# wjmaddox/online_gp

Measured on AMD Instinct MI355X. Metric: streaming updates/sec (WISKI, 50^3 inducing grid), higher is better.
Workload: dtype f32

## Files before the change

online_gp_amd/csrc/scatter_owner.h:

```cpp
#pragma once

template <typename real>
struct OwnerRec {
  static constexpr int N = 16;
};

__device__ __forceinline__ float wave_readlane(float v, int src) { return __builtin_bit_cast(float, __builtin_amdgcn_readlane(__builtin_bit_cast(int, v), src)); }
__device__ __forceinline__ int wave_readlane(int v, int src) { return __builtin_amdgcn_readlane(v, src); }
__device__ __forceinline__ double wave_readlane(double v, int src) {
  const long long b = __builtin_bit_cast(long long, v);
  const int lo = __builtin_amdgcn_readlane((int)(b & 0xffffffffll), src), hi = __builtin_amdgcn_readlane((int)(b >> 32), src);
  return __builtin_bit_cast(double, ((long long)hi << 32) | (long long)(unsigned)lo);
}
__device__ __forceinline__ void lds_atomic_add(float* p, float v) { __hip_atomic_fetch_add(p, v, __ATOMIC_RELAXED, __HIP_MEMORY_SCOPE_WORKGROUP); }
__device__ __forceinline__ void lds_atomic_add(double* p, double v) { __hip_atomic_fetch_add(p, v, __ATOMIC_RELAXED, __HIP_MEMORY_SCOPE_WORKGROUP); }

template <typename real>
static inline int64_t owner_work_bytes(const wiski_grid* g, int64_t n) {
  const int64_t ncell = (int64_t)(g->g[0] - 3) * (g->g[1] - 3) * (g->g[2] - 3);
  const int64_t heads = (ncell * 8 + 255) / 256 * 256, next = (n * 4 + 255) / 256 * 256;
  return heads + next + n * OwnerRec<real>::N * (int64_t)sizeof(real);
}

template <typename real>
__global__ __launch_bounds__(256) void k_bin_points(GridDev<real> G, const real* __restrict__ x, const real* __restrict__ y, const real* __restrict__ wa,
                                                    const real* __restrict__ wb, const real* __restrict__ noise, int64_t n,
                                                    double* __restrict__ stats, int32_t* __restrict__ err, const real* __restrict__ u, int carry,
                                                    real* __restrict__ mean_out, unsigned long long* __restrict__ head, int32_t* __restrict__ next,
                                                    real* __restrict__ rec, unsigned epoch, uint32_t* __restrict__ z1, int64_t n1,
                                                    uint32_t* __restrict__ z2, int64_t n2, const long long* __restrict__ guard, long long guard_expect) {
  if (guard && *guard != guard_expect) return;
  for (int64_t e = (int64_t)blockIdx.x * blockDim.x + threadIdx.x; e < n1; e += (int64_t)gridDim.x * blockDim.x) z1[e] = 0u;
  for (int64_t e = (int64_t)blockIdx.x * blockDim.x + threadIdx.x; e < n2; e += (int64_t)gridDim.x * blockDim.x) z2[e] = 0u;
  __shared__ double s_red[16];
  const int lane = threadIdx.x & 63, loc = threadIdx.x >> 6;
  const int nc1 = G.g[1] - 3, nc2 = G.g[2] - 3;
  bool bad = false;
  for (int64_t base = (int64_t)blockIdx.x * 4; base < n; base += (int64_t)gridDim.x * 4) {
    const int64_t p = base + loc;
    if (p >= n) continue;
    real xp[3], w[3][4];
    int j0[3];
#pragma unroll
    for (int q = 0; q < 3; ++q) xp[q] = x[p * 3 + q];
    const bool inside = point_stencil<real, 3>(G, xp, j0, w);
    if (!inside) {
      bad = true;
      if (lane == 0) {
        atomicAdd(err, 2);
        next[p] = -2;
        if (mean_out) mean_out[p] = (real)0;
      }
      continue;
    }
    const int a = lane >> 4, b = (lane >> 2) & 3, c = lane & 3;
    const real wa_ = a == 0 ? w[0][0] : a == 1 ? w[0][1] : a == 2 ? w[0][2] : w[0][3];
    const real wb_ = b == 0 ? w[1][0] : b == 1 ? w[1][1] : b == 2 ? w[1][2] : w[1][3];
    const real wc_ = c == 0 ? w[2][0] : c == 1 ? w[2][1] : c == 2 ? w[2][2] : w[2][3];
    const real v = wa_ * wb_ * wc_;
    const int64_t flat = (int64_t)(j0[0] + a) * G.stride[0] + (int64_t)(j0[1] + b) * G.stride[1] + (j0[2] + c);
    real wu = (u && v != (real)0) ? v * u[flat] : (real)0;
    if (u) wu = wave_reduce_sum<real>(wu);
    {
      real wl = (real)0;
#pragma unroll
      for (int q = 0; q < 3; ++q)
#pragma unroll
        for (int k = 0; k < 4; ++k)
          if (lane == 4 * q + k) wl = w[q][k];
      if (lane < 12) rec[p * OwnerRec<real>::N + lane] = wl;
    }
    if (lane == 12) {
      const real wap = wa[p], by = y[p] * wb[p];
      real* r = rec + p * OwnerRec<real>::N;
      r[12] = wap;
      r[13] = by;
      r[14] = carry ? by - wap * wu : (real)0;
      r[15] = (real)0;
      if (mean_out) mean_out[p] = wu;
      const int64_t cell = ((int64_t)j0[0] * nc1 + j0[1]) * nc2 + j0[2];
      const unsigned long long tag = ((unsigned long long)epoch << 32) | (unsigned long long)(unsigned)p;
      const unsigned long long old = atomicExch(head + cell, tag);
      next[p] = (unsigned)(old >> 32) == epoch ? (int32_t)(old & 0xffffffffull) : -1;
    }
  }
  scatter_stats_pass<real, 3>(G, x, y, wb, noise, n, stats, s_red);
  if (bad) atomicOr(err, 1);
}

__device__ __forceinline__ int owner_slot(int g, int s) { return g == 0 ? s - 3 : 4 + 7 * (g - 1) + s; }

template <typename real, int NT>
__global__ __launch_bounds__(NT) void k_owner_lines(GridDev<real> G, real* __restrict__ A, real* __restrict__ b, real* __restrict__ cnt,
                                                     real* __restrict__ res, const unsigned long long* __restrict__ head,
                                                     const int32_t* __restrict__ next, const real* __restrict__ rec, unsigned epoch,
                                                     const long long* __restrict__ guard, long long guard_expect, int abl) {
  if (guard && *guard != guard_expect) return;
  extern __shared__ __attribute__((aligned(16))) char smem_owner[];
  constexpr int NS = 172;
  const int g0 = G.g[0], g1 = G.g[1], g2 = G.g[2];
  const int nc0 = g0 - 3, nc1 = g1 - 3, nc2 = g2 - 3;
  const int i0 = blockIdx.x / g1, i1 = blockIdx.x % g1;
  real* acc = reinterpret_cast<real*>(smem_owner);
  real* vb = acc + (size_t)g2 * NS;
  real* vc = vb + g2;
  real* vr = vc + g2;
  __shared__ int s_any;
  const int t = threadIdx.x, lane = t & 63, wv = t >> 6;
  {
    const int nz = g2 * (NS + 3), nz4 = nz & ~3;
    for (int e = 4 * t; e < nz4; e += 4 * NT) {
      acc[e] = (real)0; acc[e + 1] = (real)0; acc[e + 2] = (real)0; acc[e + 3] = (real)0;
    }
    if (t < nz - nz4) acc[nz4 + t] = (real)0;
  }
  if (t == 0) s_any = 0;
  __syncthreads();
  const int lo = g2 * wv / (NT / 64), hi = g2 * (wv + 1) / (NT / 64);
  const int clo = lo - 3 < 0 ? 0 : lo - 3, chi = hi < nc2 ? hi : nc2;
  const int ncw = chi - clo, ncand = 16 * ncw;
  const unsigned inv_ncw = (65536u + (unsigned)ncw - 1u) / (unsigned)ncw;
  int found = 0;
  const int a = lane >> 4, bq = (lane >> 2) & 3, c = lane & 3;
  const int dummy = g2 * (NS + 3) + t;
  real m0[4], m1[4], m2[4];
#pragma unroll
  for (int k = 0; k < 4; ++k) {
    m0[k] = a == k ? (real)1 : (real)0;
    m1[k] = bq == k ? (real)1 : (real)0;
    m2[k] = c == k ? (real)1 : (real)0;
  }
  const int lcode = 7 * a + bq;
  const int lidx = 7 * lcode + c;
  auto visit = [&](real (&r)[15], int p, int da, int db, int c2) {
    const int dcode = 7 * da + db;
    const bool upper = lcode > dcode, same = lcode == dcode;
    const int abase = lidx + (c2 * NS - 7 * dcode);
    for (;;) {
      const real w0a = m0[0] * r[0] + m0[1] * r[1] + m0[2] * r[2] + m0[3] * r[3];
      const real w1b = m1[0] * r[4] + m1[1] * r[5] + m1[2] * r[6] + m1[3] * r[7];
      const real w2c = m2[0] * r[8] + m2[1] * r[9] + m2[2] * r[10] + m2[3] * r[11];
      const real w0d = da == 0 ? r[0] : da == 1 ? r[1] : da == 2 ? r[2] : r[3];
      const real w1d = db == 0 ? r[4] : db == 1 ? r[5] : db == 2 ? r[6] : r[7];
      const real wab = w0d * w1d;
      const real wj = w0a * w1b * w2c;
      const real wap = r[12];
      int ix[7];
      real add[7], cur[7];
      const real wpj = wap * wab * wj;
#pragma unroll
      for (int cr = 0; cr < 4; ++cr) {
        const bool keep = (upper || (same && c >= cr)) && c2 + cr >= lo && c2 + cr < hi;
        ix[cr] = keep ? abase + cr * (NS - 1) : dummy;
        add[cr] = wpj * r[8 + cr];
      }
      {
        const bool mine = lane < 4 && c2 + lane >= lo && c2 + lane < hi;
        const real wi = wab * w2c;
        const int row = g2 * NS + c2 + lane;
        ix[4] = mine ? row : dummy;
        ix[5] = mine ? row + g2 : dummy;
        ix[6] = mine ? row + 2 * g2 : dummy;
        add[4] = wi * r[13];
        add[5] = wi * wap;
        add[6] = wi * r[14];
      }
#pragma unroll
      for (int k = 0; k < 7; ++k) cur[k] = acc[ix[k]];
#pragma unroll
      for (int k = 0; k < 7; ++k) acc[ix[k]] = cur[k] + add[k];
      if (p < 0) break;
      const real* __restrict__ rp = rec + (int64_t)p * OwnerRec<real>::N;
#pragma unroll
      for (int k = 0; k < 15; ++k) r[k] = rp[k];
      p = next[p];
    }
  };
  constexpr int RB = sizeof(real) == 4 ? 5 : 3;
  for (int cb0 = 0; cb0 < ncand; cb0 += 64 * RB) {
    int p0[RB], nx[RB];
    real rl[RB][15];
#pragma unroll
    for (int rb = 0; rb < RB; ++rb) {
      const int ci = cb0 + 64 * rb + lane;
      p0[rb] = -1;
      if (ci < ncand) {
        const int dd = (int)(((unsigned)ci * inv_ncw) >> 16), c2 = clo + ci - dd * ncw;
        const int c0 = i0 - (dd >> 2), c1 = i1 - (dd & 3);
        if (c0 >= 0 && c0 < nc0 && c1 >= 0 && c1 < nc1) {
          const unsigned long long h = head[((int64_t)c0 * nc1 + c1) * nc2 + c2];
          if ((unsigned)(h >> 32) == epoch) p0[rb] = (int)(unsigned)(h & 0xffffffffull);
        }
      }
    }
#pragma unroll
    for (int rb = 0; rb < RB; ++rb) {
      nx[rb] = -1;
      if (p0[rb] >= 0) {
        const real* __restrict__ r = rec + (int64_t)p0[rb] * OwnerRec<real>::N;
#pragma unroll
        for (int k = 0; k < 15; ++k) rl[rb][k] = r[k];
        nx[rb] = next[p0[rb]];
      } else {
#pragma unroll
        for (int k = 0; k < 15; ++k) rl[rb][k] = (real)0;
      }
    }
#pragma unroll
    for (int rb = 0; rb < RB; ++rb) {
      unsigned long long live = __ballot(p0[rb] >= 0);
      if (abl & 1) { found |= live != 0; live = 0; }
      while (live) {
        const int src = __ffsll((long long)live) - 1;
        live &= live - 1;
        const int ci_s = cb0 + 64 * rb + src;
        const int dd = __builtin_amdgcn_readfirstlane((int)(((unsigned)ci_s * inv_ncw) >> 16));
        const int c2 = __builtin_amdgcn_readfirstlane(clo + ci_s - dd * ncw);
        found = 1;
        real r[15];
#pragma unroll
        for (int k = 0; k < 15; ++k) r[k] = wave_readlane(rl[rb][k], src);
        visit(r, wave_readlane(nx[rb], src), dd >> 2, dd & 3, c2);
      }
    }
  }
  if (found && lane == 0) s_any = 1;
  __syncthreads();
  if (!s_any || (abl & 2)) return;
  const int64_t m = G.m;
  const int64_t row0 = ((int64_t)i0 * g1 + i1) * g2;
  {
    const int n0 = 4 * g2;
    for (int e = t; e < n0; e += NT) {
      const real v = acc[(e >> 2) * NS + (e & 3)];
      if (v != (real)0) A[row0 * 4 + e] += v;
    }
  }
  const int n1 = 7 * g2;
  constexpr int NE = (448 + NT - 1) / NT;
  bool ok[NE];
  int le[NE];
#pragma unroll
  for (int j = 0; j < NE; ++j) {
    const int e = t + NT * j;
    ok[j] = e < n1;
    le[j] = (e / 7) * NS + 4 + (e % 7);
  }
  constexpr int GB = NE <= 2 ? 6 : 3;
  for (int gq = 0; gq < 24; gq += GB) {
    real v[GB][NE], o[GB][NE];
#pragma unroll
    for (int k = 0; k < GB; ++k)
#pragma unroll
      for (int j = 0; j < NE; ++j) v[k][j] = ok[j] ? acc[le[j] + 7 * (gq + k)] : (real)0;
#pragma unroll
    for (int k = 0; k < GB; ++k) {
      const real* __restrict__ Ag = A + (int64_t)(7 * (gq + k + 1) - 3) * m + row0 * 7;
#pragma unroll
      for (int j = 0; j < NE; ++j) o[k][j] = *(v[k][j] != (real)0 ? Ag + t + NT * j : A);
    }
#pragma unroll
    for (int k = 0; k < GB; ++k) {
      real* __restrict__ Ag = A + (int64_t)(7 * (gq + k + 1) - 3) * m + row0 * 7;
#pragma unroll
      for (int j = 0; j < NE; ++j)
        if (v[k][j] != (real)0) {
#ifdef WISKI_OWNER_NT_STORES
          __builtin_nontemporal_store(o[k][j] + v[k][j], Ag + t + NT * j);
#else
          Ag[t + NT * j] = o[k][j] + v[k][j];
#endif
        }
    }
  }
  for (int e = t; e < g2; e += NT) {
    if (vb[e] != (real)0) b[row0 + e] += vb[e];
    if (cnt && vc[e] != (real)0) cnt[row0 + e] += vc[e];
    if (res && vr[e] != (real)0) res[row0 + e] += vr[e];
  }
}
```

online_gp_amd/csrc/scatter_stats.hip:

```cpp
#include "wiski_common.h"

#ifndef WISKI_SCATTER_ATOMIC_MOD
#define WISKI_SCATTER_ATOMIC_MOD 0
#endif
__device__ __forceinline__ void stencil_atomic(float* p, float v) {
#if WISKI_SCATTER_ATOMIC_MOD == 1
  asm volatile("global_atomic_add_f32 %0, %1, off sc1" ::"v"(p), "v"(v) : "memory");
#elif WISKI_SCATTER_ATOMIC_MOD == 2
  asm volatile("global_atomic_add_f32 %0, %1, off nt" ::"v"(p), "v"(v) : "memory");
#elif WISKI_SCATTER_ATOMIC_MOD == 3
  asm volatile("global_atomic_add_f32 %0, %1, off sc1 nt" ::"v"(p), "v"(v) : "memory");
#else
  unsafeAtomicAdd(p, v);
#endif
}
__device__ __forceinline__ void stencil_atomic(double* p, double v) { unsafeAtomicAdd(p, v); }
#include <atomic>
#include <cstdlib>

struct ScatterBatch {
  int64_t y_stride = 0, w_stride = 0, vec_stride = 0, A_stride = 0;
};

template <typename real, int D>
__device__ __forceinline__ void scatter_stats_pass(const GridDev<real>& G, const real* __restrict__ x, const real* __restrict__ y,
                                                   const real* __restrict__ wb, const real* __restrict__ noise, int64_t n,
                                                   double* __restrict__ stats, double* s_red) {
  int64_t want = n / 512;
  want = want < 1 ? 1 : (want > 64 ? 64 : want);
  const int ns = (int64_t)gridDim.x < want ? (int)gridDim.x : (int)want;
  if ((int)blockIdx.x >= ns) return;
  double c_acc = 0, ld_acc = 0;
  for (int64_t p = (int64_t)blockIdx.x * blockDim.x + threadIdx.x; p < n; p += (int64_t)ns * blockDim.x) {
    real xp[D], w[D][4];
    int j0[D];
#pragma unroll
    for (int q = 0; q < D; ++q) xp[q] = x[p * D + q];
    if (point_stencil<real, D>(G, xp, j0, w)) {
      const double yp = (double)y[p];
      c_acc += yp * yp * (double)wb[p];
      ld_acc += log((double)noise[p]);
    }
  }
  const double c_tot = block_reduce_sum(c_acc, s_red);
  const double ld_tot = block_reduce_sum(ld_acc, s_red);
  if (threadIdx.x == 0 && (c_tot != 0 || ld_tot != 0)) {
    unsafeAtomicAdd(stats + 0, c_tot);
    unsafeAtomicAdd(stats + 1, ld_tot);
  }
}

template <typename real, int D>
__global__ __launch_bounds__(256) void k_scatter_stats(GridDev<real> G, const real* __restrict__ x, const real* __restrict__ y,
                                                       const real* __restrict__ wa, const real* __restrict__ wb,
                                                       const real* __restrict__ noise, int64_t n, real* __restrict__ b,
                                                       real* __restrict__ A_st, double* __restrict__ stats, int32_t* __restrict__ err,
                                                       real* __restrict__ cnt) {
  constexpr int T = 1 << (2 * D);
  constexpr int GRP = T < 64 ? T : 64;
  constexpr int PPB = 256 / GRP;
  constexpr int TPL = T / GRP;
  __shared__ real s_val[PPB][T];
  __shared__ double s_red[16];
  const int sub = threadIdx.x % GRP;
  const int loc = threadIdx.x / GRP;
  int R = 1;
#pragma unroll
  for (int q = 0; q < D; ++q) R *= 7;
  const int center = (R - 1) / 2;
  bool bad = false;

  for (int64_t base = (int64_t)blockIdx.x * PPB; base < n; base += (int64_t)gridDim.x * PPB) {
    const int64_t p = base + loc;
    const bool valid = p < n;
    int j0[D];
    real w[D][4];
    real yp = 0, wap = 0, wbp = 0;
    if (valid) {
      real xp[D];
#pragma unroll
      for (int q = 0; q < D; ++q) xp[q] = x[p * D + q];
      const bool inside = point_stencil<real, D>(G, xp, j0, w);
      if (!inside) {
        bad = true;
        if (sub == 0) atomicAdd(err, 2);
      }
      yp = y[p];
      wap = wa[p];
      wbp = wb[p];
    } else {
#pragma unroll
      for (int q = 0; q < D; ++q) {
        j0[q] = 0;
#pragma unroll
        for (int c = 0; c < 4; ++c) w[q][c] = 0;
      }
    }
    int idx_a[TPL], code_a[TPL];
    real val_a[TPL];
#pragma unroll
    for (int t = 0; t < TPL; ++t) {
      const int a = sub + t * GRP;
      int flat = 0, code = 0;
      real v = (real)1;
#pragma unroll
      for (int q = 0; q < D; ++q) {
        const int c = (a >> (2 * (D - 1 - q))) & 3;
        flat += (j0[q] + c) * G.stride[q];
        code = code * 7 + c;
        v *= w[q][c];
      }
      idx_a[t] = flat;
      code_a[t] = code;
      val_a[t] = v;
      s_val[loc][a] = v;
    }
    __syncthreads();
    if (valid) {
#pragma unroll
      for (int t = 0; t < TPL; ++t) {
        if (val_a[t] != (real)0) {
          atomic_add_real(b + idx_a[t], val_a[t] * yp * wbp);
          if (cnt) atomic_add_real(cnt + idx_a[t], val_a[t] * wap);
          if (A_st) {
            const real va = val_a[t] * wap;
            real* __restrict__ Arow = A_st + idx_a[t];
            const int obase = center - code_a[t];
#pragma unroll 4
            for (int bb0 = 0; bb0 < T; ++bb0) {
              const int bb = (bb0 & ~3) | ((bb0 + (sub + t * GRP)) & 3);
              int codeb = 0;
#pragma unroll
              for (int q = 0; q < D; ++q) codeb = codeb * 7 + ((bb >> (2 * (D - 1 - q))) & 3);
              const real vb = s_val[loc][bb];
              if (vb != (real)0) atomic_add_real(Arow + (int64_t)(obase + codeb) * G.m, va * vb);
            }
          }
        }
      }
    }
    __syncthreads();
  }
  scatter_stats_pass<real, D>(G, x, y, wb, noise, n, stats, s_red);
  if (bad) atomicOr(err, 1);
}

template <typename real, int D>
__global__ __launch_bounds__(256) void k_scatter_stats_sym(GridDev<real> G, const real* __restrict__ x, const real* __restrict__ y,
                                                           const real* __restrict__ wa, const real* __restrict__ wb,
                                                           const real* __restrict__ noise, int64_t n, real* __restrict__ b,
                                                           real* __restrict__ A, double* __restrict__ stats, int32_t* __restrict__ err,
                                                           real* __restrict__ cnt, const real* __restrict__ u, real* __restrict__ res,
                                                           real* __restrict__ mean_out = nullptr, uint32_t* __restrict__ z1 = nullptr,
                                                           int64_t n1 = 0, uint32_t* __restrict__ z2 = nullptr, int64_t n2 = 0,
                                                           const long long* __restrict__ guard = nullptr, long long guard_expect = 0,
                                                           int g_lo = 0, int g_hi = 1 << 30, ScatterBatch bt = ScatterBatch{}) {
  {
    const int64_t o = blockIdx.y;
    y += o * bt.y_stride; wa += o * bt.w_stride; wb += o * bt.w_stride; noise += o * bt.w_stride;
    b += o * bt.vec_stride; stats += 2 * o;
    if (A) A += o * bt.A_stride;
    if (cnt) cnt += o * bt.vec_stride;
    if (u) u += o * bt.vec_stride;
    if (res) res += o * bt.vec_stride;
  }
  if (guard && *guard != guard_expect) return;
  for (int64_t e = (int64_t)blockIdx.x * blockDim.x + threadIdx.x; e < n1; e += (int64_t)gridDim.x * blockDim.x) z1[e] = 0u;
  for (int64_t e = (int64_t)blockIdx.x * blockDim.x + threadIdx.x; e < n2; e += (int64_t)gridDim.x * blockDim.x) z2[e] = 0u;
  constexpr int T = 1 << (2 * D);
  constexpr int TP = T / 4;
  constexpr int NPAIR = TP * (TP + 1) / 2;
  constexpr int TPL = T > 64 ? T / 64 : 1;
  __shared__ real s_val[4][T];
  __shared__ int s_idx[4][T];
  __shared__ int s_pair[NPAIR];
  __shared__ int s_scan[4];
  __shared__ double s_red[16];
  const int lane = threadIdx.x & 63, loc = threadIdx.x >> 6;
  int npair = 0;
  {
    int running = 0;
    for (int base = 0; base < TP * TP; base += 256) {
      const int idx = base + threadIdx.x;
      const int pa = idx / TP, pb = idx % TP;
      int ca = 0, cb = 0;
#pragma unroll
      for (int q = 0; q < D - 1; ++q) {
        ca = ca * 7 + ((pa >> (2 * (D - 2 - q))) & 3);
        cb = cb * 7 + ((pb >> (2 * (D - 2 - q))) & 3);
      }
      const bool ok = idx < TP * TP && cb >= ca && cb - ca >= g_lo && cb - ca < g_hi;
      const unsigned long long mask = __ballot(ok);
      if (lane == 0) s_scan[loc] = __popcll(mask);
      __syncthreads();
      int off = running;
      for (int w = 0; w < loc; ++w) off += s_scan[w];
      if (ok) s_pair[off + __popcll(mask & ((1ull << lane) - 1ull))] = pa | (pb << 8) | ((cb - ca) << 16);
      running += s_scan[0] + s_scan[1] + s_scan[2] + s_scan[3];
      __syncthreads();
    }
    npair = running;
  }
  bool bad = false;
  const int64_t m = G.m;
  for (int64_t base = (int64_t)blockIdx.x * 4; base < n; base += (int64_t)gridDim.x * 4) {
    const int64_t p = base + loc;
    const bool valid = p < n;
    int j0[D];
    real w[D][4];
    real yp = 0, wap = 0, wbp = 0;
    if (valid) {
      real xp[D];
#pragma unroll
      for (int q = 0; q < D; ++q) xp[q] = x[p * D + q];
      const bool inside = point_stencil<real, D>(G, xp, j0, w);
      if (!inside) {
        bad = true;
        if (lane == 0 && blockIdx.y == 0) atomicAdd(err, 2);
      }
      yp = y[p];
      wap = wa[p];
      wbp = wb[p];
    } else {
#pragma unroll
      for (int q = 0; q < D; ++q) {
        j0[q] = 0;
#pragma unroll
        for (int c = 0; c < 4; ++c) w[q][c] = 0;
      }
    }
    int flat_t[TPL];
    real val_t[TPL];
    real wu = (real)0;
#pragma unroll
    for (int t = 0; t < TPL; ++t) {
      const int a = lane + t * 64;
      flat_t[t] = 0;
      val_t[t] = (real)0;
      if (a < T) {
        int flat = 0;
        real v = (real)1;
#pragma unroll
        for (int q = 0; q < D; ++q) {
          const int c = (a >> (2 * (D - 1 - q))) & 3;
          flat += (j0[q] + c) * G.stride[q];
          v *= w[q][c];
        }
        s_val[loc][a] = v;
        s_idx[loc][a] = flat;
        flat_t[t] = flat;
        val_t[t] = v;
        if (u && v != (real)0) wu += v * u[flat];
      }
    }
    real innov = yp * wbp;
    if (u) {
#pragma unroll
      for (int off = 32; off > 0; off >>= 1) wu += __shfl_xor(wu, off, 64);
      innov -= wap * wu;
      if (mean_out && lane == 0 && valid) mean_out[p] = wu;
    }
#pragma unroll
    for (int t = 0; t < TPL; ++t) {
      if (valid && val_t[t] != (real)0) {
        atomic_add_real(b + flat_t[t], val_t[t] * yp * wbp);
        if (cnt) atomic_add_real(cnt + flat_t[t], val_t[t] * wap);
        if (res) atomic_add_real(res + flat_t[t], val_t[t] * innov);
      }
    }
    __syncthreads();
    if (valid && A) {
      const int a2 = lane & 3, b2 = (lane >> 2) & 3, ps = lane >> 4;
#pragma unroll 2
      for (int t0 = 0; t0 < npair; t0 += 4) {
        const int t = t0 + ps;
        if (t < npair) {
          const int pk = s_pair[t];
          const int g = pk >> 16;
          const int a = (pk & 0xff) * 4 + a2;
          const real v = wap * s_val[loc][a] * s_val[loc][((pk >> 8) & 0xff) * 4 + b2];
          const int64_t row = s_idx[loc][a];
          if (g == 0) {
            if (b2 >= a2 && v != (real)0) stencil_atomic(A + row * 4 + (b2 - a2), v);
          } else if (v != (real)0) {
            stencil_atomic(A + (int64_t)(7 * g - 3) * m + row * 7 + (b2 - a2 + 3), v);
          }
        }
      }
    }
    __syncthreads();
  }
  scatter_stats_pass<real, D>(G, x, y, wb, noise, n, stats, s_red);
  if (bad) atomicOr(err, 1);
}

#include "scatter_owner.h"

template <typename real>
__global__ __launch_bounds__(256) void k_stencil_expand_add(GridDev<real> G, real* __restrict__ half, real* __restrict__ full) {
  const int m = G.m, d = G.d;
  const int c = (G.R - 1) / 2;
  const int oh = blockIdx.y;
  int rem = c + oh, off = 0;
  for (int q = d - 1; q >= 0; --q) {
    off += (rem % 7 - 3) * G.stride[q];
    rem /= 7;
  }
  const int g = oh < 4 ? 0 : (oh - 4) / 7 + 1;
  real* __restrict__ h = oh < 4 ? half + oh : half + (int64_t)(7 * g - 3) * m + (oh - 4) % 7;
  const int hs = oh < 4 ? 4 : 7;
  real* __restrict__ fd = full + (int64_t)(c + oh) * m;
  real* __restrict__ fm = full + (int64_t)(c - oh) * m;
  for (int i = blockIdx.x * blockDim.x + threadIdx.x; i < m; i += gridDim.x * blockDim.x) {
    const real v = h[(int64_t)i * hs];
    if (v != (real)0) {
      fd[i] += v;
      if (oh > 0) {
        const int j = i + off;
        if (j >= 0 && j < m) fm[j] += v;
      }
      h[(int64_t)i * hs] = (real)0;
    }
  }
}

template <typename real>
static int expand_impl(const wiski_grid* grid, real* d_half, real* d_full, void* stream) {
  GridDev<real> G;
  int rc = make_grid_dev<real>(grid, &G);
  if (rc) return rc;
  if (!d_half || !d_full) return WISKI_E_BADARG;
  int bx = (G.m + 255) / 256;
  if (bx > 64) bx = 64;
  dim3 grd((unsigned)bx, (unsigned)((G.R + 1) / 2));
  hipLaunchKernelGGL((k_stencil_expand_add<real>), grd, dim3(256), 0, (hipStream_t)stream, G, d_half, d_full);
  WISKI_LAUNCH_CHECK();
  return WISKI_OK;
}

static int64_t owner_min_points() {
  static int64_t v = -1;
  if (v < 0) {
    const char* e = getenv("WISKI_OWNER_MIN_POINTS");
    v = e ? atoll(e) : 8192;
    if (v <= 0) v = (int64_t)1 << 62;
  }
  return v;
}

static int owner_ablate() { return 0; }

template <typename real>
static int scatter_impl(const wiski_grid* grid, const real* d_x, const real* d_y, const real* d_wa, const real* d_wb, const real* d_noise,
                        int64_t n, real* d_b, real* d_A_st, double* d_stats, int32_t* d_err, void* stream, bool half = false,
                        real* d_cnt = nullptr, const real* d_u = nullptr, real* d_res = nullptr, real* d_mean_out = nullptr,
                        void* z1 = nullptr, int64_t n1_bytes = 0, void* z2 = nullptr, int64_t n2_bytes = 0, const void* d_guard = nullptr,
                        int64_t guard_expect = 0, void* d_bin = nullptr, int64_t bin_bytes = 0, int g_lo = 0, int g_hi = 1 << 30, int nout = 1,
                        ScatterBatch bt = ScatterBatch{}) {
  GridDev<real> G;
  int rc = make_grid_dev<real>(grid, &G);
  if (rc) return rc;
  if (n == 0) return WISKI_OK;
  if (!d_x || !d_y || !d_wa || !d_wb || !d_noise || !d_b || !d_stats || !d_err) return WISKI_E_BADARG;
  if (d_mean_out == nullptr && (d_u != nullptr) != (d_res != nullptr)) return WISKI_E_BADARG;
  if ((d_res && !d_u) || (d_mean_out && !d_u) || (d_u && !half)) return WISKI_E_BADARG;
  if (d_guard && !half) return WISKI_E_BADARG;
  if ((n1_bytes | n2_bytes) & 3 || (n1_bytes && !z1) || (n2_bytes && !z2) || ((n1_bytes || n2_bytes) && !half)) return WISKI_E_BADARG;
  const bool ranged = g_lo > 0 || g_hi < (1 << 30);
  if (ranged && !half) return WISKI_E_BADARG;
  if (nout < 1 || (nout > 1 && (!half || d_mean_out || n1_bytes || n2_bytes || d_guard))) return WISKI_E_BADARG;
  bool owner = !ranged && nout == 1 && half && G.d == 3 && d_bin && d_cnt && d_A_st && G.g[2] <= 64 && G.g[0] > 3 && G.g[1] > 3 && G.g[2] > 3 && n < (int64_t)1 << 31 &&
               n >= owner_min_points() && bin_bytes >= owner_work_bytes<real>(grid, n);
  const size_t owner_lds = ((size_t)G.g[2] * (172 + 3) + 512) * sizeof(real);
  if (owner) {
    static int lds_max = -1;
    static size_t lds_set = 0;
    if (lds_max < 0) {
      int dev = 0, v = 0;
      if (hipGetDevice(&dev) != hipSuccess || hipDeviceGetAttribute(&v, hipDeviceAttributeMaxSharedMemoryPerBlock, dev) != hipSuccess) v = 64 * 1024;
      lds_max = v;
    }
    if (owner_lds > (size_t)lds_max) {
      owner = false;
    } else if (owner_lds > 48 * 1024 && owner_lds > lds_set) {
      if (hipFuncSetAttribute((const void*)k_owner_lines<real, 256>, hipFuncAttributeMaxDynamicSharedMemorySize, (int)owner_lds) != hipSuccess ||
          hipFuncSetAttribute((const void*)k_owner_lines<real, 128>, hipFuncAttributeMaxDynamicSharedMemorySize, (int)owner_lds) != hipSuccess ||
          hipFuncSetAttribute((const void*)k_owner_lines<real, 512>, hipFuncAttributeMaxDynamicSharedMemorySize, (int)owner_lds) != hipSuccess) {
        (void)hipGetLastError();
        owner = false;
      } else {
        lds_set = owner_lds;
      }
    }
  }
  if (owner) {
    static std::atomic<unsigned> epoch_src{0};
    unsigned epoch = ++epoch_src;
    if (!epoch) epoch = ++epoch_src;
    const int64_t ncell = (int64_t)(G.g[0] - 3) * (G.g[1] - 3) * (G.g[2] - 3);
    char* w = static_cast<char*>(d_bin);
    unsigned long long* head = reinterpret_cast<unsigned long long*>(w);
    int32_t* next = reinterpret_cast<int32_t*>(w + (ncell * 8 + 255) / 256 * 256);
    real* rec = reinterpret_cast<real*>(w + (ncell * 8 + 255) / 256 * 256 + (n * 4 + 255) / 256 * 256);
    int64_t nb = (n + 3) / 4;
    if (nb > 2048) nb = 2048;
    hipLaunchKernelGGL((k_bin_points<real>), dim3((unsigned)nb), dim3(256), 0, (hipStream_t)stream, G, d_x, d_y, d_wa, d_wb, d_noise, n, d_stats, d_err,
                       d_u, d_res != nullptr ? 1 : 0, d_mean_out, head, next, rec, epoch, (uint32_t*)z1, n1_bytes / 4, (uint32_t*)z2, n2_bytes / 4,
                       (const long long*)d_guard, (long long)guard_expect);
    constexpr int owner_nt = 256;
    const size_t lds = owner_lds;
    const int abl = owner_ablate();
    hipLaunchKernelGGL((k_owner_lines<real, owner_nt>), dim3((unsigned)(G.g[0] * G.g[1])), dim3(owner_nt), lds, (hipStream_t)stream, G, d_A_st, d_b, d_cnt, d_res,
                       (const unsigned long long*)head, (const int32_t*)next, (const real*)rec, epoch, (const long long*)d_guard, (long long)guard_expect, abl);
    return hipGetLastError() == hipSuccess ? WISKI_OK : WISKI_E_LAUNCH;
  }
  const int grp = half ? 64 : (G.T < 64 ? G.T : 64);
  const int64_t ppb = 256 / grp;
  int64_t blocks = (n + ppb - 1) / ppb;
  if (blocks > 256 * 8) blocks = 256 * 8;
  dim3 grd((unsigned)blocks, (unsigned)nout);
#define CALL(DD)                                                                                                                              \
  do {                                                                                                                                        \
    if (half) hipLaunchKernelGGL((k_scatter_stats_sym<real, DD>), grd, dim3(256), 0, (hipStream_t)stream, G, d_x, d_y, d_wa, d_wb, d_noise, n, d_b, d_A_st, d_stats, d_err, d_cnt, d_u, d_res, d_mean_out, (uint32_t*)z1, n1_bytes / 4, (uint32_t*)z2, n2_bytes / 4, (const long long*)d_guard, (long long)guard_expect, g_lo, g_hi, bt); \
    else hipLaunchKernelGGL((k_scatter_stats<real, DD>), grd, dim3(256), 0, (hipStream_t)stream, G, d_x, d_y, d_wa, d_wb, d_noise, n, d_b, d_A_st, d_stats, d_err, d_cnt);   \
  } while (0)
  WISKI_DISPATCH_D(G.d, CALL)
#undef CALL
  WISKI_LAUNCH_CHECK();
  return WISKI_OK;
}

extern "C" {
int wiski_scatter_stats_f32(const wiski_grid* g, const float* x, const float* y, const float* wa, const float* wb, const float* noise, int64_t n, float* b, float* A, double* stats, int32_t* err, void* s) {
  return scatter_impl<float>(g, x, y, wa, wb, noise, n, b, A, stats, err, s);
}
int wiski_scatter_stats_f64(const wiski_grid* g, const double* x, const double* y, const double* wa, const double* wb, const double* noise, int64_t n, double* b, double* A, double* stats, int32_t* err, void* s) {
  return scatter_impl<double>(g, x, y, wa, wb, noise, n, b, A, stats, err, s);
}
int wiski_scatter_stats_sym_f32(const wiski_grid* g, const float* x, const float* y, const float* wa, const float* wb, const float* noise, int64_t n, float* b, float* A_half, double* stats, int32_t* err, void* s) {
  return scatter_impl<float>(g, x, y, wa, wb, noise, n, b, A_half, stats, err, s, true);
}
int wiski_scatter_stats_sym_f64(const wiski_grid* g, const double* x, const double* y, const double* wa, const double* wb, const double* noise, int64_t n, double* b, double* A_half, double* stats, int32_t* err, void* s) {
  return scatter_impl<double>(g, x, y, wa, wb, noise, n, b, A_half, stats, err, s, true);
}
int wiski_scatter_stats_cnt_f32(const wiski_grid* g, const float* x, const float* y, const float* wa, const float* wb, const float* noise, int64_t n, float* b, float* A, int32_t half, float* cnt, const float* u, float* res, double* stats, int32_t* err, void* s) {
  return scatter_impl<float>(g, x, y, wa, wb, noise, n, b, A, stats, err, s, half != 0, cnt, u, res);
}
int wiski_scatter_stats_cnt_f64(const wiski_grid* g, const double* x, const double* y, const double* wa, const double* wb, const double* noise, int64_t n, double* b, double* A, int32_t half, double* cnt, const double* u, double* res, double* stats, int32_t* err, void* s) {
  return scatter_impl<double>(g, x, y, wa, wb, noise, n, b, A, stats, err, s, half != 0, cnt, u, res);
}
int wiski_scatter_stats_step_f32(const wiski_grid* g, const float* x, const float* y, const float* wa, const float* wb, const float* noise, int64_t n, float* b, float* A_half, float* cnt, const float* u, float* res, float* mean_out, double* stats, int32_t* err, void* z1, int64_t n1, void* z2, int64_t n2, const void* guard, int64_t guard_expect, void* bin, int64_t bin_bytes, void* s) {
  return scatter_impl<float>(g, x, y, wa, wb, noise, n, b, A_half, stats, err, s, true, cnt, u, res, mean_out, z1, n1, z2, n2, guard, guard_expect, bin, bin_bytes);
}
int wiski_scatter_stats_step_f64(const wiski_grid* g, const double* x, const double* y, const double* wa, const double* wb, const double* noise, int64_t n, double* b, double* A_half, double* cnt, const double* u, double* res, double* mean_out, double* stats, int32_t* err, void* z1, int64_t n1, void* z2, int64_t n2, const void* guard, int64_t guard_expect, void* bin, int64_t bin_bytes, void* s) {
  return scatter_impl<double>(g, x, y, wa, wb, noise, n, b, A_half, stats, err, s, true, cnt, u, res, mean_out, z1, n1, z2, n2, guard, guard_expect, bin, bin_bytes);
}
int wiski_scatter_stats_step_sharded_f32(const wiski_grid* g, const float* x, const float* y, const float* wa, const float* wb, const float* noise, int64_t n, float* b, float* A_half, float* cnt, const float* u, float* res, float* mean_out, double* stats, int32_t* err, void* z1, int64_t n1, void* z2, int64_t n2, const void* guard, int64_t guard_expect, int32_t g_lo, int32_t g_hi, void* s) {
  return scatter_impl<float>(g, x, y, wa, wb, noise, n, b, A_half, stats, err, s, true, cnt, u, res, mean_out, z1, n1, z2, n2, guard, guard_expect, nullptr, 0, g_lo, g_hi);
}
int wiski_scatter_stats_step_sharded_f64(const wiski_grid* g, const double* x, const double* y, const double* wa, const double* wb, const double* noise, int64_t n, double* b, double* A_half, double* cnt, const double* u, double* res, double* mean_out, double* stats, int32_t* err, void* z1, int64_t n1, void* z2, int64_t n2, const void* guard, int64_t guard_expect, int32_t g_lo, int32_t g_hi, void* s) {
  return scatter_impl<double>(g, x, y, wa, wb, noise, n, b, A_half, stats, err, s, true, cnt, u, res, mean_out, z1, n1, z2, n2, guard, guard_expect, nullptr, 0, g_lo, g_hi);
}
int wiski_scatter_stats_multi_f32(const wiski_grid* g, const float* x, const float* y, const float* wa, const float* wb, const float* noise, int64_t n, int32_t nout, int64_t y_stride, int64_t w_stride, float* b, float* A_half, int64_t A_stride, float* cnt, const float* u, float* res, double* stats, int32_t* err, void* s) {
  ScatterBatch bt; bt.y_stride = y_stride; bt.w_stride = w_stride; bt.vec_stride = g ? (int64_t)g->g[0] * (g->d > 1 ? g->g[1] : 1) * (g->d > 2 ? g->g[2] : 1) * (g->d > 3 ? g->g[3] : 1) : 0; bt.A_stride = A_stride;
  return scatter_impl<float>(g, x, y, wa, wb, noise, n, b, A_half, stats, err, s, true, cnt, u, res, nullptr, nullptr, 0, nullptr, 0, nullptr, 0, nullptr, 0, 0, 1 << 30, nout, bt);
}
int wiski_scatter_stats_multi_f64(const wiski_grid* g, const double* x, const double* y, const double* wa, const double* wb, const double* noise, int64_t n, int32_t nout, int64_t y_stride, int64_t w_stride, double* b, double* A_half, int64_t A_stride, double* cnt, const double* u, double* res, double* stats, int32_t* err, void* s) {
  ScatterBatch bt; bt.y_stride = y_stride; bt.w_stride = w_stride; bt.vec_stride = g ? (int64_t)g->g[0] * (g->d > 1 ? g->g[1] : 1) * (g->d > 2 ? g->g[2] : 1) * (g->d > 3 ? g->g[3] : 1) : 0; bt.A_stride = A_stride;
  return scatter_impl<double>(g, x, y, wa, wb, noise, n, b, A_half, stats, err, s, true, cnt, u, res, nullptr, nullptr, 0, nullptr, 0, nullptr, 0, nullptr, 0, 0, 1 << 30, nout, bt);
}
int64_t wiski_scatter_bin_bytes(const wiski_grid* g, int64_t n, int32_t elem_size) {
  if (!g || g->d != 3 || n < 0 || (elem_size != 4 && elem_size != 8)) return -1;
  return elem_size == 4 ? owner_work_bytes<float>(g, n) : owner_work_bytes<double>(g, n);
}
int wiski_stencil_expand_add_f32(const wiski_grid* g, float* half, float* full, void* s) { return expand_impl<float>(g, half, full, s); }
int wiski_stencil_expand_add_f64(const wiski_grid* g, double* half, double* full, void* s) { return expand_impl<double>(g, half, full, s); }
}
```

Measured before the change: 25.26 million.

## Add 3D-tiled owner scatter kernel replacing per-line owner accumulation

Adds k_owner_tiles, which gives each workgroup a 4x4x13 block of grid rows. Binned points from neighbouring cells are staged through an LDS queue and accumulated into per-row stencil accumulators in LDS, then written back to global A, b, cnt and res without atomics. It replaces the per-(x,y)-line owner kernel by default, removes the g2<=64 limit, and lowers the default owner-path threshold from 8192 to 4096 points. The cost is a large LDS footprint per block and repeated queue passes over halo cells.

```diff
diff --git a/online_gp_amd/csrc/scatter_owner.h b/online_gp_amd/csrc/scatter_owner.h
--- a/online_gp_amd/csrc/scatter_owner.h
+++ b/online_gp_amd/csrc/scatter_owner.h
@@ -279,3 +279,185 @@
     if (res && vr[e] != (real)0) res[row0 + e] += vr[e];
   }
 }
+
+template <typename real>
+struct OwnerTile {
+  static constexpr int TX = sizeof(real) == 4 ? 4 : 2, TY = 4, TZ = 13;
+  static constexpr int NT = 64 * TX * TY;
+  static constexpr int NS = 172;
+  static constexpr int RW = NS + 3;
+  static constexpr int ROWS = TX * TY * TZ;
+  static constexpr int QCAP = 1024 / (int)sizeof(real);
+  static constexpr size_t ACC = (size_t)ROWS * RW * sizeof(real);
+  static constexpr size_t LDS = ACC + (size_t)QCAP * OwnerRec<real>::N * sizeof(real);
+  static_assert(ACC % 16 == 0 && LDS + 512 <= 160 * 1024, "tile accumulators and queue must fit the CU's LDS");
+};
+
+template <typename real>
+__global__ __launch_bounds__(OwnerTile<real>::NT) void k_owner_tiles(GridDev<real> G, real* __restrict__ A, real* __restrict__ b, real* __restrict__ cnt,
+                                                                     real* __restrict__ res, const unsigned long long* __restrict__ head,
+                                                                     const int32_t* __restrict__ next, const real* __restrict__ rec, unsigned epoch,
+                                                                     const long long* __restrict__ guard, long long guard_expect, int nt1, int nt2,
+                                                                     int ntiles, int abl) {
+  if (guard && *guard != guard_expect) return;
+  using TL = OwnerTile<real>;
+  constexpr int TX = TL::TX, TY = TL::TY, TZ = TL::TZ, NS = TL::NS, RW = TL::RW, NT = TL::NT, QCAP = TL::QCAP, RN = OwnerRec<real>::N;
+  extern __shared__ __attribute__((aligned(16))) char smem_owner[];
+  __shared__ int s_cnt, s_any;
+  real* acc = reinterpret_cast<real*>(smem_owner);
+  real* que = reinterpret_cast<real*>(smem_owner + TL::ACC);
+  const int per = (ntiles + 7) >> 3;
+  const int tile = (int)(blockIdx.x & 7) * per + (int)(blockIdx.x >> 3);
+  if (tile >= ntiles) return;
+  const int g0 = G.g[0], g1 = G.g[1], g2 = G.g[2];
+  const int nc0 = g0 - 3, nc1 = g1 - 3, nc2 = g2 - 3;
+  const int x0 = (tile / (nt1 * nt2)) * TX, y0 = ((tile / nt2) % nt1) * TY, z0 = (tile % nt2) * TZ;
+  const int tx = g0 - x0 < TX ? g0 - x0 : TX, ty = g1 - y0 < TY ? g1 - y0 : TY, tz = g2 - z0 < TZ ? g2 - z0 : TZ;
+  const int t = threadIdx.x, lane = t & 63, wv = t >> 6;
+  {
+    uint4* z = reinterpret_cast<uint4*>(smem_owner);
+    for (int e = t; e < (int)(TL::ACC / 16); e += NT) z[e] = make_uint4(0u, 0u, 0u, 0u);
+  }
+  if (t == 0) { s_cnt = 0; s_any = 0; }
+  const int cx0 = x0 - 3 < 0 ? 0 : x0 - 3, cy0 = y0 - 3 < 0 ? 0 : y0 - 3, cz0 = z0 - 3 < 0 ? 0 : z0 - 3;
+  const int ncx = (x0 + tx < nc0 ? x0 + tx : nc0) - cx0, ncy = (y0 + ty < nc1 ? y0 + ty : nc1) - cy0, ncz = (z0 + tz < nc2 ? z0 + tz : nc2) - cz0;
+  const int ncand = ncx * ncy * ncz;
+  constexpr int CPT = ((TX + 3) * (TY + 3) * (TZ + 3) + NT - 1) / NT;
+  int cur[CPT], code[CPT];
+#pragma unroll
+  for (int k = 0; k < CPT; ++k) {
+    const int ci = t + k * NT;
+    cur[k] = -1;
+    code[k] = 0;
+    if (ci < ncand) {
+      const int cz = ci % ncz, cxy = ci / ncz;
+      const int c0 = cx0 + cxy / ncy, c1 = cy0 + cxy % ncy, c2 = cz0 + cz;
+      code[k] = ((c0 - x0 + 3) << 16) | ((c1 - y0 + 3) << 8) | (c2 - z0 + 3);
+      const unsigned long long h = head[((int64_t)c0 * nc1 + c1) * nc2 + c2];
+      if ((unsigned)(h >> 32) == epoch) cur[k] = (int)(unsigned)(h & 0xffffffffull);
+    }
+  }
+  const int lx = wv / TY, ly = wv % TY;
+  const int a = lane >> 4, bq = (lane >> 2) & 3, c = lane & 3;
+  real m0[4], m1[4], m2[4];
+#pragma unroll
+  for (int k = 0; k < 4; ++k) {
+    m0[k] = a == k ? (real)1 : (real)0;
+    m1[k] = bq == k ? (real)1 : (real)0;
+    m2[k] = c == k ? (real)1 : (real)0;
+  }
+  const int lcode = 7 * a + bq;
+  real* accl = acc + (size_t)wv * TZ * RW;
+  for (;;) {
+    __syncthreads();
+    int more = 0;
+#pragma unroll
+    for (int k = 0; k < CPT; ++k) {
+      if (cur[k] >= 0) {
+        const int slot = atomicAdd(&s_cnt, 1);
+        if (slot < QCAP) {
+          const real* __restrict__ r = rec + (int64_t)cur[k] * RN;
+          real* q = que + slot * RN;
+#pragma unroll
+          for (int e = 0; e < RN - 1; ++e) q[e] = r[e];
+          reinterpret_cast<int*>(q + RN - 1)[0] = code[k];
+          cur[k] = next[cur[k]];
+        }
+        more |= cur[k] >= 0;
+      }
+    }
+    more = __syncthreads_or(more);
+    const int nq = s_cnt < QCAP ? s_cnt : QCAP;
+    if (nq && t == 0) s_any = 1;
+    if (!(abl & 1) && lx < tx && ly < ty) {
+      for (int k = 0; k < nq; ++k) {
+        const real* q = que + k * RN;
+        const int cd = __builtin_amdgcn_readfirstlane(reinterpret_cast<const int*>(q + RN - 1)[0]);
+        const int da = lx - ((cd >> 16) - 3), db = ly - (((cd >> 8) & 255) - 3), rz = (cd & 255) - 3;
+        if (da < 0 || da > 3 || db < 0 || db > 3) continue;
+        real r[15];
+#pragma unroll
+        for (int e = 0; e < 15; ++e) r[e] = q[e];
+        const real w0a = m0[0] * r[0] + m0[1] * r[1] + m0[2] * r[2] + m0[3] * r[3];
+        const real w1b = m1[0] * r[4] + m1[1] * r[5] + m1[2] * r[6] + m1[3] * r[7];
+        const real w2c = m2[0] * r[8] + m2[1] * r[9] + m2[2] * r[10] + m2[3] * r[11];
+        const real w0d = da == 0 ? r[0] : da == 1 ? r[1] : da == 2 ? r[2] : r[3];
+        const real w1d = db == 0 ? r[4] : db == 1 ? r[5] : db == 2 ? r[6] : r[7];
+        const real wab = w0d * w1d;
+        const real wap = r[12];
+        const real wpj = wap * wab * (w0a * w1b * w2c);
+        const int dcode = 7 * da + db;
+        const bool upper = lcode > dcode, same = lcode == dcode;
+        const int abase = rz * RW + 7 * (lcode - dcode) + c;
+        int ix[7];
+        bool keep[7];
+        real add[7], old[7];
+#pragma unroll
+        for (int cr = 0; cr < 4; ++cr) {
+          keep[cr] = (upper || (same && c >= cr)) && rz + cr >= 0 && rz + cr < tz;
+          ix[cr] = keep[cr] ? abase + cr * (RW - 1) : 0;
+          add[cr] = wpj * r[8 + cr];
+        }
+        {
+          const bool mine = lane < 4 && rz + lane >= 0 && rz + lane < tz;
+          const real wi = wab * w2c;
+          const int row = (rz + lane) * RW + NS;
+#pragma unroll
+          for (int e = 0; e < 3; ++e) {
+            keep[4 + e] = mine;
+            ix[4 + e] = mine ? row + e : 0;
+          }
+          add[4] = wi * r[13];
+          add[5] = wi * wap;
+          add[6] = wi * r[14];
+        }
+#pragma unroll
+        for (int e = 0; e < 7; ++e) old[e] = accl[ix[e]];
+#pragma unroll
+        for (int e = 0; e < 7; ++e)
+          if (keep[e]) accl[ix[e]] = old[e] + add[e];
+      }
+    }
+    if (!more) break;
+    __syncthreads();
+    if (t == 0) s_cnt = 0;
+  }
+  __syncthreads();
+  if (!s_any || (abl & 2)) return;
+  const int64_t m = G.m;
+  constexpr int SP = 7 * TZ, TOT = TX * TY * 24 * SP, WB = 7;
+  for (int e0 = 0; e0 < TOT; e0 += WB * NT) {
+    real v[WB], o[WB];
+    int64_t gi[WB];
+#pragma unroll
+    for (int k = 0; k < WB; ++k) {
+      const int e = e0 + k * NT + t;
+      const int lg = e / SP, rr = e - lg * SP, ln = lg / 24, g = lg - ln * 24 + 1, z = rr / 7, s = rr - z * 7;
+      const int ex = ln / TY, ey = ln - ex * TY;
+      const bool ok = e < TOT && ex < tx && ey < ty && z < tz;
+      v[k] = ok ? acc[((ex * TY + ey) * TZ + z) * RW + 7 * g - 3 + s] : (real)0;
+      const int64_t row = ((int64_t)(x0 + ex) * g1 + (y0 + ey)) * g2 + z0 + z;
+      gi[k] = v[k] != (real)0 ? (int64_t)(7 * g - 3) * m + row * 7 + s : 0;
+    }
+#pragma unroll
+    for (int k = 0; k < WB; ++k) o[k] = A[gi[k]];
+#pragma unroll
+    for (int k = 0; k < WB; ++k)
+      if (v[k] != (real)0) A[gi[k]] = o[k] + v[k];
+  }
+  for (int e = t; e < TX * TY * 4 * TZ; e += NT) {
+    const int ln = e / (4 * TZ), rr = e - ln * 4 * TZ, z = rr >> 2, s = rr & 3, ex = ln / TY, ey = ln - ex * TY;
+    if (ex < tx && ey < ty && z < tz) {
+      const real v = acc[((ex * TY + ey) * TZ + z) * RW + s];
+      if (v != (real)0) A[(((int64_t)(x0 + ex) * g1 + (y0 + ey)) * g2 + z0 + z) * 4 + s] += v;
+    }
+  }
+  for (int e = t; e < 3 * TL::ROWS; e += NT) {
+    const int wh = e / TL::ROWS, rw = e - wh * TL::ROWS, ln = rw / TZ, z = rw - ln * TZ, ex = ln / TY, ey = ln - ex * TY;
+    real* __restrict__ dst = wh == 0 ? b : wh == 1 ? cnt : res;
+    if (dst && ex < tx && ey < ty && z < tz) {
+      const real v = acc[rw * RW + NS + wh];
+      if (v != (real)0) dst[((int64_t)(x0 + ex) * g1 + (y0 + ey)) * g2 + z0 + z] += v;
+    }
+  }
+}
diff --git a/online_gp_amd/csrc/scatter_stats.hip b/online_gp_amd/csrc/scatter_stats.hip
--- a/online_gp_amd/csrc/scatter_stats.hip
+++ b/online_gp_amd/csrc/scatter_stats.hip
@@ -294,6 +294,9 @@
   if (bad) atomicOr(err, 1);
 }
 
+#ifndef WISKI_OWNER_MIN_POINTS_DEFAULT
+#define WISKI_OWNER_MIN_POINTS_DEFAULT 4096
+#endif
 #include "scatter_owner.h"
 
 template <typename real>
@@ -342,7 +345,7 @@
   static int64_t v = -1;
   if (v < 0) {
     const char* e = getenv("WISKI_OWNER_MIN_POINTS");
-    v = e ? atoll(e) : 8192;
+    v = e ? atoll(e) : WISKI_OWNER_MIN_POINTS_DEFAULT;
     if (v <= 0) v = (int64_t)1 << 62;
   }
   return v;
@@ -369,23 +372,34 @@
   const bool ranged = g_lo > 0 || g_hi < (1 << 30);
   if (ranged && !half) return WISKI_E_BADARG;
   if (nout < 1 || (nout > 1 && (!half || d_mean_out || n1_bytes || n2_bytes || d_guard))) return WISKI_E_BADARG;
-  bool owner = !ranged && nout == 1 && half && G.d == 3 && d_bin && d_cnt && d_A_st && G.g[2] <= 64 && G.g[0] > 3 && G.g[1] > 3 && G.g[2] > 3 && n < (int64_t)1 << 31 &&
+  bool owner = !ranged && nout == 1 && half && G.d == 3 && d_bin && d_cnt && d_A_st && G.g[0] > 3 && G.g[1] > 3 && G.g[2] > 3 && n < (int64_t)1 << 31 &&
                n >= owner_min_points() && bin_bytes >= owner_work_bytes<real>(grid, n);
+  bool tiles = owner;
   const size_t owner_lds = ((size_t)G.g[2] * (172 + 3) + 512) * sizeof(real);
+#ifdef WISKI_OWNER_FORCE_LINES
+  tiles = false;
+#endif
   if (owner) {
     static int lds_max = -1;
     static size_t lds_set = 0;
+    static int tiles_set = 0;
     if (lds_max < 0) {
       int dev = 0, v = 0;
       if (hipGetDevice(&dev) != hipSuccess || hipDeviceGetAttribute(&v, hipDeviceAttributeMaxSharedMemoryPerBlock, dev) != hipSuccess) v = 64 * 1024;
       lds_max = v;
     }
-    if (owner_lds > (size_t)lds_max) {
+    if (tiles && tiles_set == 0) {
+      tiles_set = OwnerTile<real>::LDS + 512 <= (size_t)lds_max &&
+                          hipFuncSetAttribute((const void*)k_owner_tiles<real>, hipFuncAttributeMaxDynamicSharedMemorySize, (int)OwnerTile<real>::LDS) == hipSuccess
+                      ? 1 : -1;
+      if (tiles_set < 0) (void)hipGetLastError();
+    }
+    tiles = tiles && tiles_set > 0;
+    if (tiles) {
+    } else if (G.g[2] > 64 || owner_lds > (size_t)lds_max) {
       owner = false;
     } else if (owner_lds > 48 * 1024 && owner_lds > lds_set) {
-      if (hipFuncSetAttribute((const void*)k_owner_lines<real, 256>, hipFuncAttributeMaxDynamicSharedMemorySize, (int)owner_lds) != hipSuccess ||
-          hipFuncSetAttribute((const void*)k_owner_lines<real, 128>, hipFuncAttributeMaxDynamicSharedMemorySize, (int)owner_lds) != hipSuccess ||
-          hipFuncSetAttribute((const void*)k_owner_lines<real, 512>, hipFuncAttributeMaxDynamicSharedMemorySize, (int)owner_lds) != hipSuccess) {
+      if (hipFuncSetAttribute((const void*)k_owner_lines<real, 256>, hipFuncAttributeMaxDynamicSharedMemorySize, (int)owner_lds) != hipSuccess) {
         (void)hipGetLastError();
         owner = false;
       } else {
@@ -407,6 +421,15 @@
     hipLaunchKernelGGL((k_bin_points<real>), dim3((unsigned)nb), dim3(256), 0, (hipStream_t)stream, G, d_x, d_y, d_wa, d_wb, d_noise, n, d_stats, d_err,
                        d_u, d_res != nullptr ? 1 : 0, d_mean_out, head, next, rec, epoch, (uint32_t*)z1, n1_bytes / 4, (uint32_t*)z2, n2_bytes / 4,
                        (const long long*)d_guard, (long long)guard_expect);
+    if (tiles) {
+      using TL = OwnerTile<real>;
+      const int nt0 = (G.g[0] + TL::TX - 1) / TL::TX, nt1 = (G.g[1] + TL::TY - 1) / TL::TY, nt2 = (G.g[2] + TL::TZ - 1) / TL::TZ;
+      const int64_t ntiles = (int64_t)nt0 * nt1 * nt2;
+      hipLaunchKernelGGL((k_owner_tiles<real>), dim3((unsigned)((ntiles + 7) / 8 * 8)), dim3(TL::NT), TL::LDS, (hipStream_t)stream, G, d_A_st, d_b, d_cnt,
+                         d_res, (const unsigned long long*)head, (const int32_t*)next, (const real*)rec, epoch, (const long long*)d_guard, (long long)guard_expect,
+                         nt1, nt2, (int)ntiles, owner_ablate());
+      return hipGetLastError() == hipSuccess ? WISKI_OK : WISKI_E_LAUNCH;
+    }
     constexpr int owner_nt = 256;
     const size_t lds = owner_lds;
     const int abl = owner_ablate();
```

Result: slower. 16.30 million (-35.5%).
